# finlaymiller/torch-vae

Hardware: AMD Instinct MI355X
Metric: training samples/sec (VAE step: forward+ELBO+backward+AdamW), synthetic pianoroll (higher is better)
Workload: dtype bf16; 1 GPU; VanillaVAE latent_dim=16, 128x128 synthetic pianoroll, batch 256/GPU (generalised bottleneck 256*(H/16)^2); img_size=128, latent_dim=16, batch_per_gpu=256, global_batch=256, parallelism=dp1, optimizer=AdamW+OneCycle (encoder, decoder groups)

## Files before the change

### torch_vae_amd/csrc/common.cuh

```cuda
#pragma once
#include <hip/hip_runtime.h>
#include <stdint.h>

#include "../../include/vae_step.h"

typedef __attribute__((ext_vector_type(16))) float f32x16;
typedef __attribute__((ext_vector_type(4))) float f32x4;
typedef __attribute__((ext_vector_type(2))) float f32x2;
typedef __attribute__((ext_vector_type(2))) __bf16 bf16x2;
typedef __attribute__((ext_vector_type(8))) __bf16 bf16x8;
typedef __attribute__((ext_vector_type(4))) short s16x4;
typedef __bf16 bf16;
typedef _Float16 f16;
typedef __attribute__((ext_vector_type(2))) _Float16 f16x2;
typedef __attribute__((ext_vector_type(8))) _Float16 f16x8;

#ifdef VAE_PHASE_STAMPS
#define VAE_ABLATE(word, bits) (((word) & (bits)) != 0)
#else
#define VAE_ABLATE(word, bits) false
#endif

static constexpr int WG_KP = 64;
#ifndef WG_SPAD_V
// ... 173 lines not shown
        const double sc = (double)f.gamma[c] * invstd;
        k0 = (float)sc; k1 = 0.f; k2 = (float)((double)f.beta[c] - mean * sc);
        if (invstd_out) { *invstd_out = (float)invstd; *xm_out = (float)(-mean * invstd); }
        if (writer) {
            f.block[LC_SC * C + c] = k0; f.block[LC_ZERO * C + c] = 0.f; f.block[LC_SH * C + c] = k2;
            f.block[LC_INVSTD * C + c] = (float)invstd; f.block[LC_XM * C + c] = (float)(-mean * invstd);
            f.block[LC_MEAN * C + c] = (float)mean; f.block[LC_VAR * C + c] = (float)var;
            if (f.update_running) {
                const double unb = f.count > 1 ? var * f.count / (f.count - 1) : var;
                f.running_mean[c] = (float)((1.0 - f.momentum) * f.running_mean[c] + f.momentum * mean);
                f.running_var[c] = (float)((1.0 - f.momentum) * f.running_var[c] + f.momentum * unb);
                if (c == 0 && f.nbt) f.nbt[0] += 1;
            }
        }
    } else {
        const double sdz = stat_sum(f.stat, C, c), sdzx = stat_sum(f.stat, C, C + c);
        const double invstd = f.block[LC_INVSTD * C + c], mean = f.block[LC_MEAN * C + c];
        const double s = (double)f.gamma[c] * invstd, m1 = sdz * f.inv_count, m2 = sdzx * f.inv_count;
        k0 = (float)s; k1 = (float)(-s * m2 * invstd); k2 = (float)(-s * m1 + s * m2 * mean * invstd);
        if (writer) {
            f.block[LC_P0 * C + c] = k0; f.block[LC_P1 * C + c] = k1; f.block[LC_P2 * C + c] = k2;
            f.dgamma[c] = (float)(sdzx * (double)f.ginv); f.dbeta[c] = (float)(sdz * (double)f.ginv);
            if (f.dconv_bias) f.dconv_bias[c] = 0.f;
        }
    }
}
static __global__ void bn_finalize_kernel(BnFuse f) {
    const int c = blockIdx.x * blockDim.x + threadIdx.x;
    if (c >= f.C) return;
    float k0, k1, k2;
    bn_fused_channel(f, c, true, k0, k1, k2);
}

#define HIP_CHECK_RET(expr)                                                       \
    do {                                                                          \
        hipError_t _e = (expr);                                                   \
        if (_e != hipSuccess) return vae_set_error(#expr, hipGetErrorString(_e)); \
    } while (0)
```

### torch_vae_amd/csrc/conv_mfma.cuh

```cuda
#pragma once
#include "common.cuh"

enum { EPI_FWD = 0, EPI_BWD = 1, EPI_PLAIN = 2 };

template <typename T> struct ConvArgs {
    const T* src0; const T* src1; const float* coef; float slope;
    const T* wp; const float* bias;
    T* out;
    const T* yout; const float* ocoef; float oslope;
    double* stat;
    int B, Hs, Ws, Cin, Cout;
    int lth, ltw, lTB, tiles_x, tiles_y;
    int two_src, epi;
    unsigned m_pp, m_pw, m_tx, m_txy;
    long long* dbg;
    BnFuse fuse;
    int rev, n_mt;
    int xcd;
    T* stage_out;
};

__device__ __forceinline__ int fastdiv(int x, unsigned m) { return m ? (int)__umulhi((unsigned)x, m) : x; }
static inline unsigned fastdiv_magic(int d) { return d <= 1 ? 0u : (unsigned)((0x100000000ULL + (unsigned long long)d - 1) / (unsigned long long)d); }

// ... 546 lines not shown
                        } else {
#pragma unroll
                            for (int j = 0; j < 8; ++j)
                                bf.v[j] = *reinterpret_cast<const T*>(gtile + (growbase[j] + toff) * GPITCH + (wb * 32 + r) * 2);
                        }
                    }
                    mma(acc[ti], af, bf);
                }
            }
        }
    }

    const size_t slab_id = blockIdx.x;
#pragma unroll
    for (int ti = 0; ti < NTW; ++ti) {
        const int t = ts + ti * TS;
        if (t < 9) {
#pragma unroll
            for (int i = 0; i < 16; ++i) {
                const int ca = a0 + wa * 32 + acc_row(i, lane), cb = bc0 + wb * 32 + r;
                a.slab[((slab_id * 9 + t) * CA + ca) * CB + cb] = acc[ti][i];
            }
        }
    }
}

static __global__ __launch_bounds__(256) void reduce_slab_kernel(const float* __restrict__ slab, int nslab_all, int n,
                                                                 float* __restrict__ out, int CA, int CB, float scale, int per) {
    __shared__ float part[4][64];
    const int jl = threadIdx.x & 63, g = threadIdx.x >> 6, j = blockIdx.x * 64 + jl;
    slab += (size_t)blockIdx.y * per * n; out += (size_t)blockIdx.y * n;
    const int nslab = min(per, nslab_all - (int)blockIdx.y * per);
    float s = 0.f;
    if (j < n) {
        int k = g;
        for (; k + 28 < nslab; k += 32) {
            float v[8];
#pragma unroll
            for (int u = 0; u < 8; ++u) v[u] = slab[(size_t)(k + 4 * u) * n + j];
#pragma unroll
            for (int u = 0; u < 8; ++u) s += v[u];
        }
        for (; k < nslab; k += 4) s += slab[(size_t)k * n + j];
    }
    part[g][jl] = s;
    __syncthreads();
    if (g == 0 && j < n) {
        s = (part[0][jl] + part[1][jl] + part[2][jl] + part[3][jl]) * scale;
        if (CA > 0) {
            const int t = j / (CA * CB), rem = j - t * CA * CB;
            out[(size_t)rem * 9 + t] = s;
        } else {
            out[j] = s;
        }
    }
}


template <typename T> struct ConvOutFwdMfmaArgs {
    const T* yf; const float* coef; const float* wt; const float* bias; const float* target;
    float* xhat; float* dlogit; double* accum;
    int B, H, W, n_tiles; float inv_n, slope;
    BnFuse fuse;
    int rev;
    double* part; int tB;
};

template <typename T, int RECON, bool PS = false>
__global__ __launch_bounds__(256, 2) void convout_fwd_mfma_kernel(ConvOutFwdMfmaArgs<T> a) {
    typedef typename H16<T>::v8 T8;
    constexpr int TH = 8, TW = 32, PH = TH + 2, PW = TW + 2, NP = PH * PW, NPAD = 384, PITCH = 80, NCHK = NP * 4, MAXI = 6;
    __shared__ __attribute__((aligned(16))) char atile[NPAD * PITCH];
    __shared__ float part[NPAD * 9];
    __shared__ float cf[64];
    __shared__ float wred[4];
    const int tid = threadIdx.x, lane = tid & 63, wave = tid >> 6, r = lane & 31, h = lane >> 5;
    const int tiles_x = a.W / TW, tiles_y = a.H / TH;
// ... 532 lines not shown
```

### torch_vae_amd/csrc/edge_kernels.cuh

```cuda
#pragma once
#include "common.cuh"

__device__ __forceinline__ float cg_sum(float v) {
#pragma unroll
    for (int o = 4; o < 64; o <<= 1) v += __shfl_xor(v, o, 64);
    return v;
}

template <typename T> __device__ __forceinline__ void load8(const T* p, float* o);
template <> __device__ __forceinline__ void load8<float>(const float* p, float* o) {
    f32x4 a = *reinterpret_cast<const f32x4*>(p), b = *reinterpret_cast<const f32x4*>(p + 4);
#pragma unroll
    for (int i = 0; i < 4; ++i) { o[i] = a[i]; o[4 + i] = b[i]; }
}
template <> __device__ __forceinline__ void load8<bf16>(const bf16* p, float* o) {
    bf16x8 a = *reinterpret_cast<const bf16x8*>(p);
#pragma unroll
    for (int i = 0; i < 8; ++i) o[i] = (float)a[i];
}
template <> __device__ __forceinline__ void load8<f16>(const f16* p, float* o) {
    f16x8 a = *reinterpret_cast<const f16x8*>(p);
#pragma unroll
    for (int i = 0; i < 8; ++i) o[i] = (float)a[i];
}
// ... 48 lines not shown
            win[rr][0] = rin ? left : 0.f;
#pragma unroll
            for (int e = 0; e < 4; ++e) { win[rr][1 + e] = rin ? v0[e] : 0.f; win[rr][5 + e] = rin ? v1[e] : 0.f; }
        }
#pragma unroll
        for (int u = 0; u < 4; ++u) {
            float o[8];
#pragma unroll
            for (int c = 0; c < 8; ++c) {
                float acc = br[c];
#pragma unroll
                for (int t = 0; t < 9; ++t) acc += wr[c][t] * win[t / 3][2 * u + t % 3];
                o[c] = round_as<T>(acc); s1[c] += o[c]; s2[c] += o[c] * o[c];
            }
            const size_t p = ((size_t)b * Ho + oy) * Wo + 4 * oxq + u;
            store8<T>(y + p * 32 + cg * 8, o);
        }
    }
#pragma unroll
    for (int c = 0; c < 8; ++c) {
        s1[c] = cg_sum(s1[c]); s2[c] = cg_sum(s2[c]);
        if (lane < 4) { red[wave][lane][c] = s1[c]; red[wave][lane][8 + c] = s2[c]; }
    }
    __syncthreads();
    if (tid < 64) {
        const int ch = tid & 31, k = tid >> 5;
        float s = 0.f;
#pragma unroll
        for (int wv = 0; wv < 4; ++wv) s += red[wv][ch >> 3][k * 8 + (ch & 7)];
        unsafeAtomicAdd(&stat[stat_rep() * 64 + k * 32 + ch], (double)s);
    }
}

template <typename T>
__global__ __launch_bounds__(256) void conv1_wgrad_kernel(const float* __restrict__ x, const T* __restrict__ dz,
                                                          const T* __restrict__ y, const float* __restrict__ gcoef,
                                                          float* __restrict__ slab, int B, int H, int W, BnFuse fuse) {
    __shared__ float red[4][4][72];
    const int tid = threadIdx.x, cg = tid & 3, slot = tid >> 2, lane = tid & 63, wave = tid >> 6;
    const int Ho = H >> 1, Wo = W >> 1, lw = 31 - __builtin_clz(Wo), lh = 31 - __builtin_clz(Ho);
    const int P = B * Ho * Wo;
    float p0[8], p1[8], p2[8], acc[8][9];
#pragma unroll
    for (int c = 0; c < 8; ++c) {
        if (fuse.mode == BNF_BWD) bn_fused_channel(fuse, cg * 8 + c, blockIdx.x == 0 && slot == 0, p0[c], p1[c], p2[c]);
        else { p0[c] = gcoef[cg * 8 + c]; p1[c] = gcoef[32 + cg * 8 + c]; p2[c] = gcoef[64 + cg * 8 + c]; }
#pragma unroll
        for (int t = 0; t < 9; ++t) acc[c][t] = 0.f;
    }
    const int Wq = Wo >> 2, lq = lw - 2, Q = B * Ho * Wq;
    for (int q = blockIdx.x * 64 + slot; q < Q; q += gridDim.x * 64) {
        const int oxq = q & (Wq - 1), oy = (q >> lq) & (Ho - 1), b = q >> (lq + lh);
        const int ix0 = 8 * oxq;
        float win[3][9], dv[4][8], yv[4][8];
#pragma unroll
        for (int rr = 0; rr < 3; ++rr) {
            const int iy = 2 * oy + rr - 1;
            const bool rin = iy >= 0;
            const float* row = x + ((size_t)b * H + (rin ? iy : 0)) * W + ix0;
            const f32x4 v0 = *reinterpret_cast<const f32x4*>(row), v1 = *reinterpret_cast<const f32x4*>(row + 4);
            const float left = (ix0 > 0) ? row[-1] : 0.f;
            win[rr][0] = rin ? left : 0.f;
#pragma unroll
            for (int e = 0; e < 4; ++e) { win[rr][1 + e] = rin ? v0[e] : 0.f; win[rr][5 + e] = rin ? v1[e] : 0.f; }
        }
        const size_t p0i = ((size_t)b * Ho + oy) * Wo + 4 * oxq;
#pragma unroll
        for (int u = 0; u < 4; ++u) { load8<T>(dz + (p0i + u) * 32 + cg * 8, dv[u]); load8<T>(y + (p0i + u) * 32 + cg * 8, yv[u]); }
#pragma unroll
        for (int u = 0; u < 4; ++u) {
#pragma unroll
            for (int c = 0; c < 8; ++c) {
                const float g = dv[u][c] * p0[c] + yv[u][c] * p1[c] + p2[c];
#pragma unroll
                for (int t = 0; t < 9; ++t) acc[c][t] += g * win[t / 3][2 * u + t % 3];
            }
        }
    }
#pragma unroll
    for (int c = 0; c < 8; ++c)
#pragma unroll
        for (int t = 0; t < 9; ++t) {
            const float s = cg_sum(acc[c][t]);
            if (lane < 4) red[wave][lane][c * 9 + t] = s;
        }
    __syncthreads();
    for (int j = tid; j < 288; j += 256) {
        const int t = j / 32, co = j % 32;
        float s = 0.f;
#pragma unroll
        for (int wv = 0; wv < 4; ++wv) s += red[wv][co >> 3][(co & 7) * 9 + t];
        slab[(size_t)blockIdx.x * 288 + j] = s;
    }
}

struct ConvOutArgs {
    const void* yf; const float* coef;
    const float* wt; const float* bias;
    const float* target;
    float* xhat; float* dlogit;
    double* accum;
    int B, H, W; float inv_n; float slope;
    double* part; int tB;
};

template <typename T, int RECON, bool PS = false>
__global__ __launch_bounds__(256) void convout_fwd_kernel(ConvOutArgs a) {
    constexpr int TH = 16, TW = 32, PH = TH + 2, PW = TW + 2, NP = PH * PW;
    __shared__ float part[NP * 9];
    __shared__ float wred[4];
    const int tid = threadIdx.x;
    const int tiles_x = a.W / TW, tiles_y = a.H / TH;
    const int tile = blockIdx.x, tx = tile % tiles_x, ty = (tile / tiles_x) % tiles_y, b = tile / (tiles_x * tiles_y);
    const int y0 = ty * TH, x0 = tx * TW, tb = PS ? b % a.tB : b;
    const T* yf = reinterpret_cast<const T*>(a.yf);
    for (int pix = tid; pix < NP; pix += 256) {
        const int py = pix / PW, px = pix - py * PW, gy = y0 + py - 1, gx = x0 + px - 1;
        float acc[9];
#pragma unroll
        for (int t = 0; t < 9; ++t) acc[t] = 0.f;
        if (gy >= 0 && gy < a.H && gx >= 0 && gx < a.W) {
            const T* src = yf + (((size_t)b * a.H + gy) * a.W + gx) * 32;
#pragma unroll
            for (int cgp = 0; cgp < 4; ++cgp) {
                float v[8];
// ... 779 lines not shown
```

### torch_vae_amd/csrc/vae_api.hip

```cpp
#include <map>
#include <mutex>
#include "vae_ctx.h"
#include "edge_kernels.cuh"
#include "loglik.cuh"
#include "latent_stats.cuh"
#include "grad_clip.cuh"

static thread_local std::string g_err;
int vae_set_error(const char* what, const char* why) {
    g_err = std::string(what) + ": " + why;
    return -1;
}

extern "C" const char* vae_last_error(void) { return g_err.c_str(); }
extern "C" int vae_abi_version(void) { return 1; }

static void param_shapes(int H, int L, int gen, int64_t* sizes) {
    const int s = gen ? H / 16 : 2;
    const int64_t F = 256LL * s * s;
    const int enc_ci[4] = {1, 32, 64, 128}, enc_co[4] = {32, 64, 128, 256};
    int k = 0;
    for (int i = 0; i < 4; ++i) { sizes[k++] = 9LL * enc_ci[i] * enc_co[i]; sizes[k++] = enc_co[i]; sizes[k++] = enc_co[i]; sizes[k++] = enc_co[i]; }
    sizes[k++] = L * F; sizes[k++] = L; sizes[k++] = L * F; sizes[k++] = L; sizes[k++] = F * L; sizes[k++] = F;
    const int dec_ci[3] = {256, 128, 64}, dec_co[3] = {128, 64, 32};
// ... 53 lines not shown
    (void)vae_comm_destroy(c);
    for (void* p : c->allocs) (void)hipFree(p);
    if (c->ll_kb) (void)hipFree(c->ll_kb);
    if (c->n_side_ok) {
        for (int i = 0; i < vae_ctx::NSIDE; ++i) { (void)hipStreamSynchronize(c->side[i]); (void)hipEventDestroy(c->ev_join[i]); }
        (void)hipStreamSynchronize(c->comm);
        for (int i = 0; i < vae_ctx::NFORK; ++i) (void)hipEventDestroy(c->ev_fork[i]);
        (void)hipEventDestroy(c->ev_pack); (void)hipEventDestroy(c->ev_comm);
        if (c->ev_kl) (void)hipEventDestroy(c->ev_kl);
        for (int i = 0; i < vae_ctx::NBUCKET; ++i) (void)hipEventDestroy(c->ev_bucket[i]);
    }
    delete c;
}
extern "C" int64_t vae_workspace_bytes(const vae_ctx* c) { return c ? c->ws_bytes : 0; }

extern "C" vae_ctx* vae_create(int H, int L, int maxB, int dtype, int gen) {
    vae_ctx* c = new vae_ctx();
    c->H = H; c->L = L; c->maxB = maxB; c->dtype = dtype; c->gen = gen; c->ws_bytes = 0; c->use_tr16 = 1; c->use_mfma_convout = 1; c->use_pipelined = 1; c->knob_up_per_cu = 2; c->knob_convout_grid = 1536; c->knob_convout_bwd_grid = 1024; c->knob_down_per_cu = 2; c->knob_nt_max = 4; c->knob_pipe_max_cout = 256; c->knob_ablate_b = 0; c->use_side_stream = 1; c->knob_bwd_per_cu = 0; c->knob_wave_nt_max = 4; c->knob_lay22_min_nt = 2; c->knob_down_waves = 8; c->knob_pack_grid = 128; c->knob_xcd_map = 1; c->knob_up_nt_max = 1; c->knob_lay42 = 1; c->knob_wgrad_layer_wgs = 0; c->knob_conv1_grid = 512; c->use_fused_bn = 1; c->knob_rev = 4; c->knob_lean = 1; c->walk_dir = 0; c->n_side_ok = 0; c->side_rr = 0; c->fork_rr = 0; c->comm_busy = 0; c->dbg_buf = nullptr; c->dbg_tag[0] = 0; c->dbg_epi = 0;
    if (getenv("VAE_NO_SIDE_STREAM")) c->use_side_stream = 0;
    c->packed_for = nullptr; c->bwd_dirty = 1; c->bwd_half_done = 0; c->B = 0; c->trained = 0; c->prof = 0; c->tag = nullptr;
    if (vae_param_layout(H, L, gen, c->poff, c->psz, &c->ptotal) != 0) { delete c; return nullptr; }
    if (dtype != VAE_DTYPE_F32 && dtype != VAE_DTYPE_BF16 && dtype != VAE_DTYPE_F16) { vae_set_error("vae_create", "bad dtype"); delete c; return nullptr; }
    c->gmul = 1.f; c->ginv = 1.f; c->generic_accum = nullptr;
    if (maxB < 1) { vae_set_error("vae_create", "max_batch < 1"); delete c; return nullptr; }
    vae_bn_layout(c->bnoff, c->bnc, &c->bntotal);
    c->s = gen ? H / 16 : 2; c->s2 = c->s * c->s; c->F = 256LL * c->s2;
    c->npad_fc = (int)align_up(2 * L, 32); c->npad_di = (int)align_up(L, 32);
    c->esz = dtype == VAE_DTYPE_F32 ? 4 : 2;
    const size_t B = maxB;
    const int hs[8] = {H / 2, H / 4, H / 8, H / 16, 2 * c->s, 4 * c->s, 8 * c->s, 16 * c->s};
    size_t nd = 0;
    for (int i = 0; i < 8; ++i) nd += 4 * kBnC[i];
    nd *= STAT_R;
    c->n_dstats = nd + 8 * STAT_R;
    c->dstats = dalloc<double>(c, c->n_dstats);
    bool ok = c->dstats != nullptr;
    double* dp = c->dstats;
    for (int i = 0; i < 8 && ok; ++i) {
        BnLayer& l = c->lay[i];
        l.C = kBnC[i]; l.H = hs[i]; l.W = hs[i];
        l.stat_f = dp; dp += 2 * l.C * STAT_R;
        const size_t n = B * l.H * l.W * l.C;
        l.y = dalloc<char>(c, n * c->esz); l.dz = dalloc<char>(c, n * c->esz); l.block = dalloc<float>(c, LC_ROWS * l.C);
        ok = l.y && l.dz && l.block;
        const int base = i < 4 ? 4 * i : (i < 7 ? 22 + 4 * (i - 4) : 34);
        l.p_convw = base; l.p_convb = base + 1; l.p_gamma = base + 2; l.p_beta = base + 3;
    }
    for (int i = 0; i < 8; ++i) { c->lay[i].stat_b = dp; dp += 2 * kBnC[i] * STAT_R; }
    c->accum = dp;
    if (ok) {
        c->d0 = dalloc<char>(c, B * c->F * c->esz); c->dd0 = dalloc<char>(c, B * c->F * c->esz);
        c->eps = dalloc<float>(c, B * L); c->dlat = dalloc<float>(c, B * 2 * L);
        c->dlogit = dalloc<float>(c, B * H * H); c->dlogit2 = dalloc<float>(c, B * H * H); c->ident = dalloc<float>(c, 3 * 256); c->wout_t = dalloc<float>(c, 288);
        ok = c->d0 && c->dd0 && c->eps && c->dlat && c->dlogit && c->dlogit2 && c->ident && c->wout_t;
    }
    const int ci[8] = {1, 32, 64, 128, 256, 128, 64, 32}, co[8] = {32, 64, 128, 256, 128, 64, 32, 32};
    for (int i = 1; i < 8 && ok; ++i) {
        const size_t n = (size_t)9 * ci[i] * co[i];
        c->wp_fwd[i] = dalloc<char>(c, n * c->esz); c->wp_dg[i] = dalloc<char>(c, n * c->esz);
        ok = c->wp_fwd[i] && c->wp_dg[i];
    }
    if (ok) {
        c->fcpack = dalloc<char>(c, (size_t)c->F * c->npad_fc * c->esz);
        c->dipack = dalloc<char>(c, (size_t)c->F * c->npad_di * c->esz);
        c->d_descs = dalloc<PackDesc>(c, 32);
        ok = c->fcpack && c->dipack && c->d_descs;
    }
    size_t slab = 2048 * 288;
    if (ok) {
        int a, b2, wa, wb;
        for (int wide = 0; wide < 2; ++wide)
            for (int big = 0; big < 2; ++big) {
                if (wide && dtype == VAE_DTYPE_F32) continue;
                for (int i = 1; i < 4; ++i) slab = std::max(slab, wgrad_slab_floats(c->wk, maxB, c->lay[i].H, c->lay[i].W, co[i], ci[i], &a, &b2, &wa, &wb, wide != 0, big != 0));
                for (int i = 4; i < 8; ++i) slab = std::max(slab, wgrad_slab_floats(c->wk, maxB, c->lay[i].H / 2, c->lay[i].W / 2, ci[i], co[i], &a, &b2, &wa, &wb, wide != 0, big != 0));
            }
        const size_t ksteps = c->F / 16;
        slab = std::max(slab, (size_t)std::min<size_t>(ksteps, 512) * maxB * c->npad_fc);
        slab = std::max(slab, (size_t)std::min<size_t>(ksteps, 512) * maxB * c->npad_di);
        slab = std::max(slab, (size_t)8 * (2 * (size_t)L * c->F + c->F));
        c->slab_floats = slab;
// ... 35 lines not shown
    for (int i = 0; i < 256; ++i) id[i] = 1.f;
    if (hipMemcpy(c->ident, id.data(), id.size() * 4, hipMemcpyHostToDevice) != hipSuccess) { vae_set_error("vae_create", "memcpy failed"); vae_destroy(c); return nullptr; }
    return c;
}

extern "C" int vae_set_option(vae_ctx* c, const char* name, int value) {
    if (!c) return vae_set_error("vae_set_option", "null ctx");
    if (!strcmp(name, "use_tr16")) { c->use_tr16 = value; return 0; }
    if (!strcmp(name, "use_mfma_convout")) { c->use_mfma_convout = value; return 0; }
    if (!strcmp(name, "use_pipelined")) { c->use_pipelined = value; return 0; }
    if (!strcmp(name, "knob_up_per_cu")) { c->knob_up_per_cu = value; return 0; }
    if (!strcmp(name, "knob_convout_grid")) { c->knob_convout_grid = value; return 0; }
    if (!strcmp(name, "knob_down_per_cu")) { c->knob_down_per_cu = std::max(1, value); return 0; }
    if (!strcmp(name, "knob_convout_bwd_grid")) { c->knob_convout_bwd_grid = value; return 0; }
    if (!strcmp(name, "knob_nt_max")) { c->knob_nt_max = value; return 0; }
    if (!strcmp(name, "knob_pipe_max_cout")) { c->knob_pipe_max_cout = value; return 0; }
    if (!strcmp(name, "knob_ablate_b")) { c->knob_ablate_b = value; return 0; }
    if (!strcmp(name, "use_side_stream")) { c->use_side_stream = value; return 0; }
    if (!strcmp(name, "knob_bwd_per_cu")) { c->knob_bwd_per_cu = value; return 0; }
    if (!strcmp(name, "knob_wave_nt_max")) { c->knob_wave_nt_max = value; return 0; }
    if (!strcmp(name, "use_fused_bn")) { c->use_fused_bn = value; return 0; }
    if (!strcmp(name, "knob_lay22_min_nt")) { c->knob_lay22_min_nt = value; return 0; }
    if (!strcmp(name, "knob_down_waves")) { c->knob_down_waves = value; return 0; }
    if (!strcmp(name, "knob_wgrad_layer_wgs")) { c->knob_wgrad_layer_wgs = value; return 0; }
    if (!strcmp(name, "knob_lay42")) { c->knob_lay42 = value; return 0; }
    if (!strcmp(name, "knob_up_nt_max")) { c->knob_up_nt_max = value < 1 ? 1 : value; return 0; }
    if (!strcmp(name, "knob_xcd_map")) { c->knob_xcd_map = value; return 0; }
    if (!strcmp(name, "knob_pack_grid")) { c->knob_pack_grid = value > 0 ? value : 1; return 0; }
    if (!strcmp(name, "knob_conv1_grid")) { c->knob_conv1_grid = value; return 0; }
    if (!strcmp(name, "knob_rev")) { c->knob_rev = value; return 0; }
    if (!strcmp(name, "knob_lean")) { c->knob_lean = value; return 0; }
    if (!strcmp(name, "use_fused_wgrad")) { c->use_fused_wgrad = value == 1 ? 3 : (value == 2 ? 1 : (value == 3 ? 2 : 0)); return 0; }
    if (!strcmp(name, "use_recomp_dz")) { c->use_recomp_dz = value; return 0; }
    if (!strcmp(name, "use_fc_dgrad8")) { c->use_fc_dgrad8 = value; return 0; }
    if (!strcmp(name, "use_fused_convout")) { c->use_fused_convout = value; return 0; }
    if (!strcmp(name, "use_convout_stream")) { c->use_convout_stream = value; return 0; }
    if (!strcmp(name, "use_wgrad_split")) { c->use_wgrad_split = value; return 0; }
    if (!strcmp(name, "use_upf_stream")) { c->use_upf_stream = value; return 0; }
    if (!strcmp(name, "use_dnf_stream")) { c->use_dnf_stream = value; return 0; }
    if (!strcmp(name, "knob_convout_bands")) { c->knob_convout_bands = value; return 0; }
    if (!strcmp(name, "knob_convout_step_grid")) { c->knob_convout_step_grid = value > 0 ? value : 1; return 0; }
    if (!strcmp(name, "knob_ablate_f")) { c->knob_ablate_f = value; return 0; }
    if (!strcmp(name, "knob_skip_wgrad")) { c->knob_skip_wgrad = value; return 0; }
    if (!strcmp(name, "use_raw_wgrad")) { c->use_raw_wgrad = value; return 0; }
    if (!strcmp(name, "use_deep")) { c->use_deep = value; return 0; }
    if (!strcmp(name, "use_latent_mfma")) { c->use_latent_mfma = value; return 0; }
    if (!strcmp(name, "knob_fused_grid")) { c->knob_fused_grid = std::max(1, std::min(value, 512)); return 0; }
    if (!strcmp(name, "knob_wgrad_tile")) { c->wk.tile = value; return 0; }
    if (!strcmp(name, "knob_wgrad_wide")) { c->wk.wide = value; return 0; }
    if (!strcmp(name, "knob_wgrad_mid8")) { c->wk.mid8 = value; return 0; }
    if (!strcmp(name, "knob_wgrad_force_simple")) { c->wk.force_simple = value; return 0; }
    if (!strcmp(name, "knob_wgrad_wide_wgs")) { c->wk.wide_wgs = std::min(value, 1024); return 0; }
    if (!strcmp(name, "knob_wgrad_wgs")) { c->wk.wgs = std::min(value, 1024); return 0; }
    if (!strcmp(name, "knob_wgrad_cap_mb")) { c->wk.cap_mb = std::min(value, 48); return 0; }
    return vae_set_error("vae_set_option", "unknown option");
}
SideFork fork_side(vae_ctx* c, hipStream_t st, int which) {
    SideFork f{st, c->slab, 0};
    if (!c->use_side_stream) return f;
    const int s = which >= 0 ? which : (c->side_rr++ % vae_ctx::NSIDE);
    hipEvent_t ev = c->ev_fork[c->fork_rr++ % vae_ctx::NFORK];
    if (hipEventRecord(ev, st) != hipSuccess || hipStreamWaitEvent(c->side[s], ev, 0) != hipSuccess) {
        f.rc = vae_set_error("fork_side", "event record/wait failed"); return f;
    }
    f.st = c->side[s]; f.slab = c->side_slab[s];
    return f;
// ... 769 lines not shown
```

### torch_vae_amd/csrc/vae_ctx.h

```cpp
#pragma once
#include <hip/hip_runtime.h>
#include <stdio.h>
#include <string.h>
#include <math.h>
#include <string>
#include <vector>
#include <algorithm>

#include "../../include/vae_step.h"

int vae_set_error(const char* what, const char* why);

#include "common.cuh"

#define LAUNCH_CHECK(name)                                                        \
    do {                                                                          \
        hipError_t _e = hipGetLastError();                                        \
        if (_e != hipSuccess) return vae_set_error(name, hipGetErrorString(_e)); \
    } while (0)

static const int kBnC[8] = {32, 64, 128, 256, 128, 64, 32, 32};
static const float kSlope = 0.01f;
static const float kBnEps = 1e-5f;
static const float kBnMom = 0.1f;
// ... 11 lines not shown
struct BnLayer {
    int C, H, W;
    double* stat_f; double* stat_b; float* block; void* y; void* dz;
    int p_gamma, p_beta, p_convw, p_convb;
    void* act = nullptr; void* dy = nullptr; int act_ok = 0, dy_ok = 0;
};

struct PackDesc {
    const float* src; const float* src2; void* dst;
    int kind;
    int A, Bc, k_is_first, npad, L, s2;
    long n;
};

struct WgradKnobs { int wgs = 128, cap_mb = 48, tile = 1, wide = 1, wide_wgs = 128, small_wgs = 1024, mid8 = 0, force_simple = 0; };

struct vae_ctx {
    int H, L, maxB, dtype, gen, s, s2; int64_t F; int npad_fc, npad_di; size_t esz;
    int64_t poff[VAE_NUM_PARAMS], psz[VAE_NUM_PARAMS], ptotal, bnoff[8], bnc[8], bntotal;
    BnLayer lay[8];
    void *d0, *dd0;
    float *eps, *dlat, *dlogit, *dlogit2, *ident, *wout_t;
    void* wp_fwd[8]; void* wp_dg[8];
    void *fcpack, *dipack;
    PackDesc* d_descs; std::vector<PackDesc> h_descs; const float* packed_for;
    float* slab; size_t slab_floats;
    static constexpr int NSIDE = 3, NFORK = 16;
    hipStream_t side[NSIDE]; float* side_slab[NSIDE]; hipEvent_t ev_fork[NFORK], ev_join[NSIDE], ev_pack; int side_rr, fork_rr, n_side_ok;
    static constexpr int NBUCKET = 2; hipEvent_t ev_bucket[NBUCKET];
    hipStream_t comm; hipEvent_t ev_comm; int comm_busy;
    void* nccl_comm = nullptr; int comm_rank = 0, comm_world = 0;
    int use_side_stream, knob_bwd_per_cu, knob_wave_nt_max, knob_lay22_min_nt, knob_down_waves, knob_pack_grid, knob_xcd_map, knob_up_nt_max, knob_lay42, knob_wgrad_layer_wgs, knob_conv1_grid, use_fused_bn, knob_rev, knob_lean, walk_dir, bwd_dirty, bwd_half_done;
    double* dstats; size_t n_dstats; double* accum;
    double* generic_accum;
    WgradKnobs wk;
    float* reduce_tmp = nullptr; size_t reduce_tmp_floats = 0; unsigned reduce_slot = 0;
    float* fused_slab[3] = {nullptr, nullptr, nullptr}; size_t fused_slab_floats = 0;
    int use_raw_wgrad = 0;
    int use_deep = 1;
    int use_latent_mfma = 6;
    int knob_skip_wgrad = 0;
    int knob_ablate_f = 0;
    int use_fused_convout = 1, convout_pending = 0, dlogit_valid = 0;
    int use_dnf_stream = 1;
    int use_upf_stream = 1;
    int use_fc_dgrad8 = 1;
    int use_wgrad_split = 1;
    int use_convout_stream = 1, knob_convout_bands = 0;
    int knob_convout_step_grid = 1024;
    BnFuse pending_f7; float* loss_out3 = nullptr; float loss_kw = 0.f;
    int recon = VAE_RECON_BCE, fwd_recon = VAE_RECON_BCE;
    int kl_kind = VAE_KL_PLAIN, fwd_kl_kind = VAE_KL_PLAIN; double kl_param = 0.0, fwd_kl_param = 0.0;
    static constexpr int KL_SIDE = 2;
    void* kl_ws = nullptr; unsigned* kl_tk = nullptr; hipEvent_t ev_kl = nullptr; int kl_pending = 0;
    unsigned long long* kl_d() const { return static_cast<unsigned long long*>(kl_ws); }
    double* kl_scal() const { return reinterpret_cast<double*>(kl_d() + L); }
    float* kl_factor() const { return reinterpret_cast<float*>(kl_scal() + 2); }
    const double* kl_shaped() const { return fwd_kl_kind != VAE_KL_PLAIN ? kl_scal() : nullptr; }
    double* ps_part = nullptr; int ps_tb = 0, ps_ntile = 0;
    float* ll_f = nullptr; double* ll_part = nullptr; double* ll_lat = nullptr;
    double* ll_kb = nullptr; size_t ll_kb_n = 0;
    int use_fused_wgrad = 3, knob_fused_grid = 256, use_recomp_dz = 0;
    float gmul, ginv;
    int B; int trained; int fwd_kind = 0; const float* x; float *xhat, *mu, *lv, *z;
    int use_tr16, use_mfma_convout, use_pipelined, knob_up_per_cu, knob_convout_grid, knob_convout_bwd_grid, knob_down_per_cu, knob_nt_max, knob_pipe_max_cout, knob_ablate_b; long long* dbg_buf; char dbg_tag[32]; int dbg_epi; int64_t ws_bytes;
    std::vector<void*> allocs;
// ... 84 lines not shown
```

### torch_vae_amd/csrc/vae_impl.cuh

```cuda
#pragma once
#include "vae_ctx.h"
#include "conv_mfma.cuh"
#include "conv_pipe.cuh"
#include "edge_kernels.cuh"
#include "conv_fused.cuh"
#include "conv_deep.cuh"
#include "latent_mfma.cuh"
#include "convout_stream.cuh"
#include "wgrad_split.cuh"
#include "upfinal_stream.cuh"
#include "dnfirst_stream.cuh"
#include "grad_paths.cuh"

template <typename K> static int set_lds(K kernel, size_t bytes) {
    if (bytes > 160 * 1024) return vae_set_error("lds", "tile needs more than 160 KiB LDS");
    if (bytes > 48 * 1024) {
        hipError_t e = hipFuncSetAttribute(reinterpret_cast<const void*>(kernel), hipFuncAttributeMaxDynamicSharedMemorySize, (int)bytes);
        if (e != hipSuccess) return vae_set_error("hipFuncSetAttribute", hipGetErrorString(e));
    }
    return 0;
}

template <typename T> static int launch_conv_pipe(vae_ctx* c, ConvArgs<T> a, bool is_down, hipStream_t st);
template <typename T> static bool fits_i32(const ConvArgs<T>& a) { return 4.0 * a.B * a.Hs * a.Ws * std::max(a.Cin, a.Cout) * sizeof(T) < 4294967296.0 && 4.0 * a.B * a.Hs * a.Ws * std::max(a.Cin, a.Cout) < 2147483648.0; }
// ... 642 lines not shown
        a.yprev = reinterpret_cast<const T*>(lp.y); a.ocoef = lp.block; a.dzprev = reinterpret_cast<T*>(lp.dz); a.stat = lp.stat_b;
        a.slab = c->fused_slab[2]; a.slope = kSlope; a.B = c->B; a.Hs = Hs; a.Ws = Ws; a.rev = (c->knob_rev >> 2) & 1; a.ablate = c->knob_ablate_f;
        const size_t lds = conv_fused_lds();
        const double px = (double)c->B * Hs * Ws;
        {
            ProfScope ps(c, "conv_bwd_fused(dgrad+wgrad)", sizeof(T) * (2.0 * px * 64 + 2.0 * 4 * px * 32 + 9.0 * 32 * 64) + 4.0 * 9 * 32 * 64,
                         2.0 * 2 * 9 * 32 * 64 * px, st);
            if (set_lds(conv_bwd_fused_kernel<T>, lds)) return -1;
            hipLaunchKernelGGL((conv_bwd_fused_kernel<T>), dim3(grid), dim3(512), lds, st, a);
            LAUNCH_CHECK("conv_bwd_fused_kernel");
        }
        SideFork f = fork_side(c, st);
        if (f.rc) return -1;
        if (launch_reduce(a.slab, grid, (size_t)9 * 64 * 32, grads + c->poff[l.p_convw], 64, 32, f.st, c)) return -1;
        return 0;
    }
}

template <typename T>
static int wgrad_on_side(vae_ctx* c, WgradArgs<T> w, float* dw_out, hipStream_t st, bool raw = false) {
    SideFork f = fork_side(c, st);
    if (f.rc) return f.rc;
    return launch_wgrad<T>(c, w, dw_out, f.st, f.slab, raw);
}
template <typename T>
static bool raw_wgrad_ok(vae_ctx* c, int i) {
    return sizeof(T) == 2 && c->use_raw_wgrad && c->use_pipelined && c->wk.wide && c->wk.tile == 1 && !c->wk.force_simple && i >= 2 && i <= 5;
}

static int bwd_clear_stats(vae_ctx* c, hipStream_t st) {
    size_t nfwd = 0;
    for (int i = 0; i < 8; ++i) nfwd += 2 * kBnC[i] * STAT_R;
    if (c->bwd_dirty) {
        HIP_CHECK_RET(hipMemsetAsync(c->dstats + nfwd, 0, nfwd * sizeof(double), st));
        for (int rep = 0; rep < STAT_R; ++rep) HIP_CHECK_RET(hipMemsetAsync(c->accum + rep * 8 + 2, 0, sizeof(double), st));
    }
    c->bwd_dirty = 1;
    return 0;
}

template <typename T>
static int backward_first(vae_ctx* c, const float* x, const float* params, float* grads, const float* g_xhat, const float* gscale,
                         const float* g_mu, const float* g_lv, const float* g_z, const float* g_pre, float kld_weight, int add_kl,
                         hipStream_t st, bool ex = false) {
    if (!c->B || !(c->trained || ex)) return vae_set_error("vae_backward", "no train-mode forward to differentiate");
    const int B = c->B, H = c->H, L = c->L;
    if (bwd_clear_stats(c, st)) return -1;
    const float* dl_src = c->dlogit; const float* dl_scale = gscale;
    const bool step7 = c->convout_pending != 0;
    if (step7 && (g_xhat || gscale || !add_kl)) return vae_set_error("vae_backward", "the forward ran with train = 2: only the standard ELBO backward (no upstream gradient on xhat, no loss scale) can follow");
    if (!step7 && add_kl && !c->dlogit_valid) return vae_set_error("vae_backward", "this forward's output-conv gradient was already consumed (train = 2 forwards can be differentiated once)");
    if (g_xhat || !add_kl) {
        const long n = (long)B * H * H;
        hipLaunchKernelGGL(dlogit_combine_kernel, dim3((unsigned)std::min<long>((n + 255) / 256, 4096)), dim3(256), 0, st,
                           g_xhat, c->xhat, add_kl ? c->dlogit : nullptr, gscale, c->dlogit2, n);
        LAUNCH_CHECK("dlogit_combine_kernel");
        dl_src = c->dlogit2; dl_scale = nullptr;
    }
    static const char* kLayerTag[8] = {"encoder.0", "encoder.1", "encoder.2", "encoder.3", "decoder.0", "decoder.1", "decoder.2", "final_layer.0"};
    c->tag = "final_layer.3";
    int cgrid = 0;
    bool recomp7 = false;
    {
        ConvOutBwdArgs a;
        a.yf = c->lay[7].y; a.ocoef = c->lay[7].block; a.wt = c->wout_t; a.dlogit = dl_src; a.gscale = dl_scale;
        a.dz = c->lay[7].dz; a.slab = c->use_side_stream ? c->side_slab[0] : c->slab; a.stat = c->lay[7].stat_b; a.dbias = c->accum + 2; a.B = B; a.H = H; a.W = H; a.slope = kSlope;
        a.gmul = c->gmul;
// ... 263 lines not shown
        if (i == 1) {
            const int rc = launch_conv_fused<T>(c, i, params, grads, st);
            if (rc < 0) return -1;
            if (rc == 0) continue;
        }
        const BnLayer& l = c->lay[i]; const BnLayer& lp = c->lay[i - 1];
        WgradArgs<T> w; memset(&w, 0, sizeof(w));
        w.s0 = reinterpret_cast<const T*>(l.dz); w.s1 = reinterpret_cast<const T*>(l.y); w.scoef = l.block + LC_P0 * l.C; w.sslope = 1.f; w.s_two = 1;
        w.g0 = reinterpret_cast<const T*>(lp.y); w.gcoef = lp.block; w.gslope = kSlope; w.g_two = 0;
        w.B = B; w.Hs = l.H; w.Ws = l.W; w.CA = l.C; w.CB = lp.C;
        ConvArgs<T> a; memset(&a, 0, sizeof(a));
        a.src0 = reinterpret_cast<const T*>(l.dz); a.src1 = reinterpret_cast<const T*>(l.y); a.coef = l.block + LC_P0 * l.C; a.slope = 1.f; a.two_src = 1;
        a.wp = reinterpret_cast<const T*>(c->wp_dg[i]);
        a.out = reinterpret_cast<T*>(lp.dz); a.yout = reinterpret_cast<const T*>(lp.y); a.ocoef = lp.block; a.oslope = kSlope; a.stat = lp.stat_b; a.epi = EPI_BWD;
        a.B = B; a.Hs = l.H; a.Ws = l.W; a.Cin = l.C; a.Cout = lp.C;
        BnFuse fb = make_fuse_bwd(c, i, params, grads);
        if (!(c->use_fused_bn && will_pipe(c, a)) || !c->trained) { if (bn_bwd_standalone(c, fb, st)) return -1; }
        w.fuse = fb; a.fuse = fb;
        const bool raw = raw_wgrad_ok<T>(c, i) && l.dy && will_pipe(c, a) && lp.act_ok;
        if (raw) {
            a.stage_out = reinterpret_cast<T*>(l.dy);
            if (launch_up<T>(c, a, st)) return -1;
            w.s0 = reinterpret_cast<const T*>(l.dy); w.s1 = nullptr; w.s_two = 0; w.sslope = 1.f;
            w.g0 = reinterpret_cast<const T*>(lp.act); w.g1 = nullptr; w.g_two = 0; w.gslope = 1.f; w.fuse.mode = BNF_NONE;
            if (!((c->knob_skip_wgrad >> i) & 1) && wgrad_on_side<T>(c, w, grads + c->poff[l.p_convw], st, true)) return -1;
            continue;
        }
        if (!((c->knob_skip_wgrad >> i) & 1) && wgrad_on_side<T>(c, w, grads + c->poff[l.p_convw], st)) return -1;
        if (launch_up<T>(c, a, st)) return -1;
    }
    {
        c->tag = kLayerTag[0];
        BnFuse fb0 = make_fuse_bwd(c, 0, params, grads);
        if (!c->use_fused_bn || !(c->knob_lean & 2) || !c->trained) { if (bn_bwd_standalone(c, fb0, st)) return -1; }
        const long P = (long)B * (H / 2) * (H / 2);
        const int grid = (int)std::min<long>((P / 4 + 63) / 64, 512);
        SideFork f{st, c->slab, 0};
        {
            ProfScope ps(c, "conv1_wgrad", 4.0 * B * H * H + (double)sizeof(T) * 64.0 * P, 2.0 * 9 * 32 * P, f.st);
            hipLaunchKernelGGL((conv1_wgrad_kernel<T>), dim3(grid), dim3(256), 0, f.st, x, reinterpret_cast<const T*>(c->lay[0].dz),
                               reinterpret_cast<const T*>(c->lay[0].y), c->lay[0].block + LC_P0 * 32, f.slab, B, H, H, fb0);
            LAUNCH_CHECK("conv1_wgrad_kernel");
        }
        if (launch_reduce(f.slab, grid, 288, grads + c->poff[0], 32, 1, f.st, c)) return -1;
        if (out) {
            if (P >= (1L << 31)) return vae_set_error("vae_backward_ex", "input gradient: batch too large for 32-bit pixel indices");
            const long Q = (P + 63) / 64;
            ProfScope ps(c, "conv1_dgrad", (double)sizeof(T) * 64.0 * P + 4.0 * B * H * H, 2.0 * 9 * 32 * P, st);
            hipLaunchKernelGGL((conv1_dgrad_kernel<T>), dim3((unsigned)std::min<long>(Q, 2048)), dim3(256), 0, st, reinterpret_cast<const T*>(c->lay[0].dz),
                               reinterpret_cast<const T*>(c->lay[0].y), c->lay[0].block + LC_P0 * 32, params + c->poff[0], out, B, H, H, c->ginv);
            LAUNCH_CHECK("conv1_dgrad_kernel");
        }
    }
    return join_sides(c, st);
}

template <typename T>
int backward_impl(vae_ctx* c, const float* x, const float* params, float* grads, const float* g_xhat, const float* gscale,
                         const float* g_mu, const float* g_lv, const float* g_z, const float* g_pre, float kld_weight, int add_kl,
                         int part, hipStream_t st) {
    if (part < 0 || part > 2) return vae_set_error("vae_backward", "part must be 0, 1 or 2");
    if (c->fwd_kind != 0 && c->B) return vae_set_error("vae_backward", "the last forward ran the encoder or the decoder only: use vae_backward_ex");
    if (part != 2) {
        if (backward_first<T>(c, x, params, grads, g_xhat, gscale, g_mu, g_lv, g_z, g_pre, kld_weight, add_kl, st)) return -1;
        c->bwd_half_done = 1;
        if (part == 1) return join_sides(c, st);
    } else if (!c->bwd_half_done) return vae_set_error("vae_backward", "part 2 before part 1");
    c->bwd_half_done = 0;
    if (backward_second<T>(c, x, params, grads, gscale, g_mu, g_lv, g_z, g_pre, kld_weight, add_kl, st)) return -1;
    return join_comm(c, st);
}

template <typename T>
int backward_ex_impl(vae_ctx* c, const float* x, const float* params, float* grads, const float* g_xhat, const float* gscale,
                     const float* g_mu, const float* g_lv, const float* g_z, const float* g_pre, float kld_weight, int add_kl,
                     float* dx, float* dz, hipStream_t st) {
    if (!c->B) return vae_set_error("vae_backward_ex", "no forward to differentiate");
// ... 34 lines not shown
```

Baseline: 235,600 samples/s.

## Recompute conv1 output in wgrad and fuse slab reduction via last-arriver tail

The first-layer weight-gradient kernel now recomputes the conv1 pre-BN output from the input window and weights held in LDS, instead of loading y from memory. It computes the BN backward coefficients once per block into LDS, and folds the slab reduction into the same kernel with atomic tickets (two-level last-arriver), which removes the separate reduce launch. This trades extra FLOPs and a serialized tail in the last block for fewer bytes read and one fewer kernel launch. Rounding is matched to the forward through selective non-contracted multiplies.

```diff
diff --git a/torch_vae_amd/csrc/common.cuh b/torch_vae_amd/csrc/common.cuh
--- a/torch_vae_amd/csrc/common.cuh
+++ b/torch_vae_amd/csrc/common.cuh
@@ -229,6 +229,60 @@
     bn_fused_channel(f, c, true, k0, k1, k2);
 }
 
+template <int M>
+__device__ __forceinline__ void slab_chains(const float* slab, int nslab, int n, const int (&j)[M], const int (&g)[M], float (&s)[M]) {
+    int kb = 0;
+#pragma unroll
+    for (int m = 0; m < M; ++m) s[m] = 0.f;
+    for (; kb + 31 < nslab; kb += 32) {
+        float v[M][8];
+#pragma unroll
+        for (int m = 0; m < M; ++m)
+#pragma unroll
+            for (int u = 0; u < 8; ++u) v[m][u] = j[m] >= 0 ? slab[(size_t)(kb + g[m] + 4 * u) * n + j[m]] : 0.f;
+#pragma unroll
+        for (int m = 0; m < M; ++m)
+#pragma unroll
+            for (int u = 0; u < 8; ++u) s[m] += v[m][u];
+    }
+    float v[M][8];
+#pragma unroll
+    for (int m = 0; m < M; ++m)
+#pragma unroll
+        for (int u = 0; u < 8; ++u) {
+            const int k = kb + g[m] + 4 * u;
+            v[m][u] = (j[m] >= 0 && k < nslab) ? slab[(size_t)k * n + j[m]] : 0.f;
+        }
+#pragma unroll
+    for (int m = 0; m < M; ++m)
+#pragma unroll
+        for (int u = 0; u < 8; ++u) s[m] = kb + g[m] + 4 * u < nslab ? s[m] + v[m][u] : s[m];
+}
+__device__ __forceinline__ float slab_chain(const float* slab, int nslab, int n, int j, int g) {
+    const int jj[1] = {j}, gg[1] = {g};
+    float s[1];
+    slab_chains<1>(slab, nslab, n, jj, gg, s);
+    return s[0];
+}
+__device__ __forceinline__ bool last_arriver(unsigned* ticket, unsigned count, float* flag) {
+    asm volatile("s_waitcnt vmcnt(0)" ::: "memory");
+    __syncthreads();
+    if (threadIdx.x == 0) {
+        __builtin_amdgcn_fence(__ATOMIC_RELEASE, "agent");
+        asm volatile("s_waitcnt vmcnt(0)" ::: "memory");
+        const unsigned t = __hip_atomic_fetch_add(ticket, 1u, __ATOMIC_RELAXED, __HIP_MEMORY_SCOPE_AGENT);
+        const bool last = t == count - 1;
+        if (last) {
+            __builtin_amdgcn_fence(__ATOMIC_ACQUIRE, "agent");
+            asm volatile("s_waitcnt vmcnt(0)" ::: "memory");
+            __hip_atomic_store(ticket, 0u, __ATOMIC_RELAXED, __HIP_MEMORY_SCOPE_AGENT);
+        }
+        *flag = last ? 1.f : 0.f;
+    }
+    __syncthreads();
+    return *flag != 0.f;
+}
+
 #define HIP_CHECK_RET(expr)                                                       \
     do {                                                                          \
         hipError_t _e = (expr);                                                   \
diff --git a/torch_vae_amd/csrc/conv_mfma.cuh b/torch_vae_amd/csrc/conv_mfma.cuh
--- a/torch_vae_amd/csrc/conv_mfma.cuh
+++ b/torch_vae_amd/csrc/conv_mfma.cuh
@@ -602,17 +602,7 @@
     slab += (size_t)blockIdx.y * per * n; out += (size_t)blockIdx.y * n;
     const int nslab = min(per, nslab_all - (int)blockIdx.y * per);
     float s = 0.f;
-    if (j < n) {
-        int k = g;
-        for (; k + 28 < nslab; k += 32) {
-            float v[8];
-#pragma unroll
-            for (int u = 0; u < 8; ++u) v[u] = slab[(size_t)(k + 4 * u) * n + j];
-#pragma unroll
-            for (int u = 0; u < 8; ++u) s += v[u];
-        }
-        for (; k < nslab; k += 4) s += slab[(size_t)k * n + j];
-    }
+    if (j < n) s = slab_chain(slab, nslab, n, j, g);
     part[g][jl] = s;
     __syncthreads();
     if (g == 0 && j < n) {
diff --git a/torch_vae_amd/csrc/edge_kernels.cuh b/torch_vae_amd/csrc/edge_kernels.cuh
--- a/torch_vae_amd/csrc/edge_kernels.cuh
+++ b/torch_vae_amd/csrc/edge_kernels.cuh
@@ -104,27 +104,74 @@
     }
 }
 
-template <typename T>
-__global__ __launch_bounds__(256) void conv1_wgrad_kernel(const float* __restrict__ x, const T* __restrict__ dz,
+template <typename T> __device__ constexpr unsigned conv1_fwd_split(int u, int c) {
+    return c >= 6 ? (u == 0 ? 0x60u : 0x6Cu) : 0u;
+}
+__device__ __forceinline__ f32x2 mul_rounded(f32x2 a, f32x2 b) {
+#pragma clang fp contract(off)
+    return a * b;
+}
+__device__ __forceinline__ float mul_rounded(float a, float b) {
+#pragma clang fp contract(off)
+    return a * b;
+}
+__device__ __forceinline__ float conv1_bn_grad(float dz, float y, float p0, float p1, float p2) {
+    return __builtin_fmaf(dz, p0, mul_rounded(y, p1)) + p2;
+}
+template <typename T> __device__ __forceinline__ f32x2 conv1_tap(f32x2 a, f32x2 w, float xv, int u, int c, int t) {
+    const f32x2 x2 = {xv, xv};
+    return (conv1_fwd_split<T>(u, c) >> t & 1) ? a + mul_rounded(w, x2) : __builtin_elementwise_fma(w, x2, a);
+}
+struct Conv1Tail {
+    float* part;
+    float* out;
+    unsigned* ticket;
+    int per;
+    float scale;
+};
+
+__device__ __forceinline__ void conv1_tail_chains(const float* slab, int nslab, float* red) {
+    int j[5], g[5]; float s[5];
+#pragma unroll
+    for (int m = 0; m < 5; ++m) { const int i = threadIdx.x + 256 * m; j[m] = i < 1152 ? i % 288 : -1; g[m] = i / 288; }
+    slab_chains<5>(slab, nslab, 288, j, g, s);
+#pragma unroll
+    for (int m = 0; m < 5; ++m) if (j[m] >= 0) red[threadIdx.x + 256 * m] = s[m];
+}
+
+template <typename T, bool RECOMP>
+__global__ __launch_bounds__(256) __attribute__((amdgpu_waves_per_eu(2))) void conv1_wgrad_kernel(const float* __restrict__ x, const T* __restrict__ dz,
                                                           const T* __restrict__ y, const float* __restrict__ gcoef,
-                                                          float* __restrict__ slab, int B, int H, int W, BnFuse fuse) {
-    __shared__ float red[4][4][72];
+                                                          const float* __restrict__ w, const float* __restrict__ bias,
+                                                          float* slab, int B, int H, int W, BnFuse fuse, Conv1Tail tail) {
+    __shared__ __attribute__((aligned(16))) float red[4 * 4 * 72 + 4 + 96 + (RECOMP ? 32 * 12 : 0)];
     const int tid = threadIdx.x, cg = tid & 3, slot = tid >> 2, lane = tid & 63, wave = tid >> 6;
     const int Ho = H >> 1, Wo = W >> 1, lw = 31 - __builtin_clz(Wo), lh = 31 - __builtin_clz(Ho);
     const int P = B * Ho * Wo;
     float p0[8], p1[8], p2[8], acc[8][9];
+    float* plds = red + 1156;
+    float* wlds = red + 1252;
+    if constexpr (RECOMP) {
+        for (int i = tid; i < 32 * 12; i += 256) {
+            const int ch = i / 12, k = i - ch * 12;
+            wlds[i] = k < 9 ? w[ch * 9 + k] : (k == 9 ? bias[ch] : 0.f);
+        }
+    }
+    if (fuse.mode == BNF_BWD && tid < 32) bn_fused_channel(fuse, tid, blockIdx.x == 0, plds[tid], plds[32 + tid], plds[64 + tid]);
+    if (RECOMP || fuse.mode == BNF_BWD) __syncthreads();
 #pragma unroll
     for (int c = 0; c < 8; ++c) {
-        if (fuse.mode == BNF_BWD) bn_fused_channel(fuse, cg * 8 + c, blockIdx.x == 0 && slot == 0, p0[c], p1[c], p2[c]);
-        else { p0[c] = gcoef[cg * 8 + c]; p1[c] = gcoef[32 + cg * 8 + c]; p2[c] = gcoef[64 + cg * 8 + c]; }
+        const float* pc = fuse.mode == BNF_BWD ? plds : gcoef;
+        p0[c] = pc[cg * 8 + c]; p1[c] = pc[32 + cg * 8 + c]; p2[c] = pc[64 + cg * 8 + c];
 #pragma unroll
         for (int t = 0; t < 9; ++t) acc[c][t] = 0.f;
     }
     const int Wq = Wo >> 2, lq = lw - 2, Q = B * Ho * Wq;
     for (int q = blockIdx.x * 64 + slot; q < Q; q += gridDim.x * 64) {
+        if constexpr (RECOMP) asm volatile("" ::: "memory");
         const int oxq = q & (Wq - 1), oy = (q >> lq) & (Ho - 1), b = q >> (lq + lh);
         const int ix0 = 8 * oxq;
-        float win[3][9], dv[4][8], yv[4][8];
+        float win[3][9], dv[4][8], yv[RECOMP ? 1 : 4][8];
 #pragma unroll
         for (int rr = 0; rr < 3; ++rr) {
             const int iy = 2 * oy + rr - 1;
@@ -138,14 +185,45 @@
         }
         const size_t p0i = ((size_t)b * Ho + oy) * Wo + 4 * oxq;
 #pragma unroll
-        for (int u = 0; u < 4; ++u) { load8<T>(dz + (p0i + u) * 32 + cg * 8, dv[u]); load8<T>(y + (p0i + u) * 32 + cg * 8, yv[u]); }
-#pragma unroll
         for (int u = 0; u < 4; ++u) {
-#pragma unroll
-            for (int c = 0; c < 8; ++c) {
-                const float g = dv[u][c] * p0[c] + yv[u][c] * p1[c] + p2[c];
-#pragma unroll
-                for (int t = 0; t < 9; ++t) acc[c][t] += g * win[t / 3][2 * u + t % 3];
+            load8<T>(dz + (p0i + u) * 32 + cg * 8, dv[u]);
+            if constexpr (!RECOMP) load8<T>(y + (p0i + u) * 32 + cg * 8, yv[u]);
+        }
+        if constexpr (RECOMP) {
+#pragma unroll
+            for (int cp = 0; cp < 4; ++cp) {
+                f32x2 wr[9], br;
+                {
+                    const f32x4* wq = reinterpret_cast<const f32x4*>(wlds + (cg * 8 + 2 * cp) * 12);
+                    const f32x4 a0 = wq[0], a1 = wq[1], a2 = wq[2], b0 = wq[3], b1 = wq[4], b2 = wq[5];
+#pragma unroll
+                    for (int e = 0; e < 4; ++e) { wr[e] = f32x2{a0[e], b0[e]}; wr[4 + e] = f32x2{a1[e], b1[e]}; }
+                    wr[8] = f32x2{a2[0], b2[0]}; br = f32x2{a2[1], b2[1]};
+                }
+#pragma unroll
+                for (int u = 0; u < 4; ++u) {
+                    f32x2 a = br;
+#pragma unroll
+                    for (int t = 0; t < 9; ++t) a = conv1_tap<T>(a, wr[t], win[t / 3][2 * u + t % 3], u, 2 * cp, t);
+                    const float yc[2] = {round_as<T>(a.x), round_as<T>(a.y)};
+#pragma unroll
+                    for (int k = 0; k < 2; ++k) {
+                        const int c = 2 * cp + k;
+                        const float g = conv1_bn_grad(dv[u][c], yc[k], p0[c], p1[c], p2[c]);
+#pragma unroll
+                        for (int t = 0; t < 9; ++t) acc[c][t] += g * win[t / 3][2 * u + t % 3];
+                    }
+                }
+            }
+        } else {
+#pragma unroll
+            for (int u = 0; u < 4; ++u) {
+#pragma unroll
+                for (int c = 0; c < 8; ++c) {
+                    const float g = conv1_bn_grad(dv[u][c], yv[u][c], p0[c], p1[c], p2[c]);
+#pragma unroll
+                    for (int t = 0; t < 9; ++t) acc[c][t] += g * win[t / 3][2 * u + t % 3];
+                }
             }
         }
     }
@@ -154,15 +232,36 @@
 #pragma unroll
         for (int t = 0; t < 9; ++t) {
             const float s = cg_sum(acc[c][t]);
-            if (lane < 4) red[wave][lane][c * 9 + t] = s;
+            if (lane < 4) red[(wave * 4 + lane) * 72 + c * 9 + t] = s;
         }
     __syncthreads();
     for (int j = tid; j < 288; j += 256) {
         const int t = j / 32, co = j % 32;
         float s = 0.f;
 #pragma unroll
-        for (int wv = 0; wv < 4; ++wv) s += red[wv][co >> 3][(co & 7) * 9 + t];
+        for (int wv = 0; wv < 4; ++wv) s += red[(wv * 4 + (co >> 3)) * 72 + (co & 7) * 9 + t];
         slab[(size_t)blockIdx.x * 288 + j] = s;
+    }
+    if (tail.out) {
+        const int nslab = gridDim.x;
+        const float* src = slab; int cnt = nslab;
+        if (tail.per) {
+            const int grp = blockIdx.x / tail.per, ngrp = (nslab + tail.per - 1) / tail.per;
+            cnt = min(tail.per, nslab - grp * tail.per);
+            if (!last_arriver(tail.ticket + grp, cnt, &red[1152])) return;
+            conv1_tail_chains(slab + (size_t)grp * tail.per * 288, cnt, red);
+            __syncthreads();
+            for (int j = tid; j < 288; j += 256) tail.part[grp * 288 + j] = red[j] + red[288 + j] + red[576 + j] + red[864 + j];
+            if (grp == ngrp - 1) for (int i = ngrp * 288 + tid; i < 32 * 288; i += 256) tail.part[i] = 0.f;
+            src = tail.part; cnt = 32;
+        }
+        if (!last_arriver(tail.ticket + 32, tail.per ? (nslab + tail.per - 1) / tail.per : nslab, &red[1152])) return;
+        conv1_tail_chains(src, cnt, red);
+        __syncthreads();
+        for (int j = tid; j < 288; j += 256) {
+            const int t = j / 32, co = j % 32;
+            tail.out[co * 9 + t] = (red[j] + red[288 + j] + red[576 + j] + red[864 + j]) * tail.scale;
+        }
     }
 }
 
diff --git a/torch_vae_amd/csrc/vae_api.hip b/torch_vae_amd/csrc/vae_api.hip
--- a/torch_vae_amd/csrc/vae_api.hip
+++ b/torch_vae_amd/csrc/vae_api.hip
@@ -109,7 +109,7 @@
     size_t nd = 0;
     for (int i = 0; i < 8; ++i) nd += 4 * kBnC[i];
     nd *= STAT_R;
-    c->n_dstats = nd + 8 * STAT_R;
+    c->n_dstats = nd + vae_ctx::kTailTicketDoubles + 8 * STAT_R;
     c->dstats = dalloc<double>(c, c->n_dstats);
     bool ok = c->dstats != nullptr;
     double* dp = c->dstats;
@@ -124,6 +124,7 @@
         l.p_convw = base; l.p_convb = base + 1; l.p_gamma = base + 2; l.p_beta = base + 3;
     }
     for (int i = 0; i < 8; ++i) { c->lay[i].stat_b = dp; dp += 2 * kBnC[i] * STAT_R; }
+    c->tail_tk = reinterpret_cast<unsigned*>(dp); dp += vae_ctx::kTailTicketDoubles;
     c->accum = dp;
     if (ok) {
         c->d0 = dalloc<char>(c, B * c->F * c->esz); c->dd0 = dalloc<char>(c, B * c->F * c->esz);
@@ -225,6 +226,7 @@
     if (!strcmp(name, "knob_lean")) { c->knob_lean = value; return 0; }
     if (!strcmp(name, "use_fused_wgrad")) { c->use_fused_wgrad = value == 1 ? 3 : (value == 2 ? 1 : (value == 3 ? 2 : 0)); return 0; }
     if (!strcmp(name, "use_recomp_dz")) { c->use_recomp_dz = value; return 0; }
+    if (!strcmp(name, "use_conv1_recomp")) { c->use_conv1_recomp = value; return 0; }
     if (!strcmp(name, "use_fc_dgrad8")) { c->use_fc_dgrad8 = value; return 0; }
     if (!strcmp(name, "use_fused_convout")) { c->use_fused_convout = value; return 0; }
     if (!strcmp(name, "use_convout_stream")) { c->use_convout_stream = value; return 0; }
diff --git a/torch_vae_amd/csrc/vae_ctx.h b/torch_vae_amd/csrc/vae_ctx.h
--- a/torch_vae_amd/csrc/vae_ctx.h
+++ b/torch_vae_amd/csrc/vae_ctx.h
@@ -67,6 +67,8 @@
     void* nccl_comm = nullptr; int comm_rank = 0, comm_world = 0;
     int use_side_stream, knob_bwd_per_cu, knob_wave_nt_max, knob_lay22_min_nt, knob_down_waves, knob_pack_grid, knob_xcd_map, knob_up_nt_max, knob_lay42, knob_wgrad_layer_wgs, knob_conv1_grid, use_fused_bn, knob_rev, knob_lean, walk_dir, bwd_dirty, bwd_half_done;
     double* dstats; size_t n_dstats; double* accum;
+    static constexpr int kTailTicketDoubles = 32;
+    int use_conv1_recomp = 1; unsigned* tail_tk = nullptr;
     double* generic_accum;
     WgradKnobs wk;
     float* reduce_tmp = nullptr; size_t reduce_tmp_floats = 0; unsigned reduce_slot = 0;
diff --git a/torch_vae_amd/csrc/vae_impl.cuh b/torch_vae_amd/csrc/vae_impl.cuh
--- a/torch_vae_amd/csrc/vae_impl.cuh
+++ b/torch_vae_amd/csrc/vae_impl.cuh
@@ -698,7 +698,7 @@
     size_t nfwd = 0;
     for (int i = 0; i < 8; ++i) nfwd += 2 * kBnC[i] * STAT_R;
     if (c->bwd_dirty) {
-        HIP_CHECK_RET(hipMemsetAsync(c->dstats + nfwd, 0, nfwd * sizeof(double), st));
+        HIP_CHECK_RET(hipMemsetAsync(c->dstats + nfwd, 0, (nfwd + vae_ctx::kTailTicketDoubles) * sizeof(double), st));
         for (int rep = 0; rep < STAT_R; ++rep) HIP_CHECK_RET(hipMemsetAsync(c->accum + rep * 8 + 2, 0, sizeof(double), st));
     }
     c->bwd_dirty = 1;
@@ -1028,17 +1028,40 @@
     {
         c->tag = kLayerTag[0];
         BnFuse fb0 = make_fuse_bwd(c, 0, params, grads);
-        if (!c->use_fused_bn || !(c->knob_lean & 2) || !c->trained) { if (bn_bwd_standalone(c, fb0, st)) return -1; }
+        const bool tail_on = c->use_conv1_recomp != 0, recomp = tail_on && sizeof(T) == 2;
+        if (!c->use_fused_bn || !(tail_on || (c->knob_lean & 2)) || !c->trained) { if (bn_bwd_standalone(c, fb0, st)) return -1; }
         const long P = (long)B * (H / 2) * (H / 2);
         const int grid = (int)std::min<long>((P / 4 + 63) / 64, 512);
         SideFork f{st, c->slab, 0};
+        const T* dz0 = reinterpret_cast<const T*>(c->lay[0].dz); const T* y0 = reinterpret_cast<const T*>(c->lay[0].y);
+        const float* gc0 = c->lay[0].block + LC_P0 * 32;
+        Conv1Tail tail; memset(&tail, 0, sizeof(tail));
+        if (tail_on) {
+            constexpr int G = 32; constexpr size_t kSlot = 16384;
+            tail.out = grads + c->poff[0]; tail.ticket = c->tail_tk; tail.scale = c->ginv;
+            if (grid >= 256 && (size_t)288 * 32 * 4 <= c->reduce_tmp_floats) {
+                tail.per = (grid + G - 1) / G;
+                tail.part = c->reduce_tmp + (size_t)(c->reduce_slot++ % (c->reduce_tmp_floats / kSlot)) * kSlot;
+            }
+        }
         {
-            ProfScope ps(c, "conv1_wgrad", 4.0 * B * H * H + (double)sizeof(T) * 64.0 * P, 2.0 * 9 * 32 * P, f.st);
-            hipLaunchKernelGGL((conv1_wgrad_kernel<T>), dim3(grid), dim3(256), 0, f.st, x, reinterpret_cast<const T*>(c->lay[0].dz),
-                               reinterpret_cast<const T*>(c->lay[0].y), c->lay[0].block + LC_P0 * 32, f.slab, B, H, H, fb0);
+            const double slab_bytes = tail_on ? 4.0 * 288 * (2.0 * grid + 1) : 0.0;
+            ProfScope ps(c, "conv1_wgrad", 4.0 * B * H * H + (double)sizeof(T) * (recomp ? 32.0 : 64.0) * P + slab_bytes,
+                         2.0 * 9 * 32 * P * (recomp ? 2 : 1), f.st);
+            bool launched = false;
+            if constexpr (sizeof(T) == 2) {
+                if (recomp) {
+                    hipLaunchKernelGGL((conv1_wgrad_kernel<T, true>), dim3(grid), dim3(256), 0, f.st, x, dz0, y0, gc0,
+                                       params + c->poff[0], params + c->poff[1], f.slab, B, H, H, fb0, tail);
+                    launched = true;
+                }
+            }
+            if (!launched)
+                hipLaunchKernelGGL((conv1_wgrad_kernel<T, false>), dim3(grid), dim3(256), 0, f.st, x, dz0, y0, gc0,
+                                   (const float*)nullptr, (const float*)nullptr, f.slab, B, H, H, fb0, tail);
             LAUNCH_CHECK("conv1_wgrad_kernel");
         }
-        if (launch_reduce(f.slab, grid, 288, grads + c->poff[0], 32, 1, f.st, c)) return -1;
+        if (!tail_on && launch_reduce(f.slab, grid, 288, grads + c->poff[0], 32, 1, f.st, c)) return -1;
         if (out) {
             if (P >= (1L << 31)) return vae_set_error("vae_backward_ex", "input gradient: batch too large for 32-bit pixel indices");
             const long Q = (P + 63) / 64;
```

Measured after the change: 236,500 samples/s (median of 5 runs). About the same (+0.4%).
